# kakaobrain/hqtransformer

Measured on AMD Instinct MI355X. Metric: images/sec (256x256 class-cond sampling), higher is better.
Workload: dtype bf16

## Files before the change

hqtransformer_amd/csrc/common.h:

```cpp
#pragma once
#include <hip/hip_runtime.h>
#include <stdint.h>
#include <string>

typedef uint16_t bf16_t;

__device__ __host__ inline float bf16_to_f32(bf16_t v) {
    union { uint32_t u; float f; } c;
    c.u = ((uint32_t)v) << 16;
    return c.f;
}
__device__ __forceinline__ void bf16x8_to_f32(const uint4& raw, float (&f)[8]) {
    const unsigned w[4] = {raw.x, raw.y, raw.z, raw.w};
#pragma unroll
    for (int i = 0; i < 4; ++i) { f[2 * i] = bf16_to_f32((bf16_t)(w[i] & 0xffffu)); f[2 * i + 1] = bf16_to_f32((bf16_t)(w[i] >> 16)); }
}
__device__ __host__ inline bf16_t f32_to_bf16(float f) {
#if defined(__HIP_DEVICE_COMPILE__)
    return __builtin_bit_cast(bf16_t, (__bf16)f);
#endif
    union { uint32_t u; float f; } c;
    c.f = f;
    if ((c.u & 0x7fffffffu) > 0x7f800000u) return (bf16_t)((c.u >> 16) | 0x40);
    return (bf16_t)((c.u + 0x7fffu + ((c.u >> 16) & 1u)) >> 16);
// ... 87 lines not shown
    float alpha;
    int store;
    int rows_per_group;
    int group_stride;
    int row_offset;
    const int* row_offset_dev;
    int rows_per_image;
    int clamp01;
    void* C2;
    void* C3;
    int qkv_D;
    int qkv_first;
    bf16_t* qkv_v_pk;
    int c_packed_mb;
    const void* zero_page;
    const float* ln_parts;
    int ln_nparts;
    const float* ln_colsum;
    float ln_eps;
    bf16_t* resid_pk;
    float* resid_parts;
    unsigned* tile_ctr;
    const float* am_rownorm;
    const float* am_colnorm;
    unsigned long long* am_best;
    ChainSync chain;
    float* gn_part_out;
    int gn_out_groups;
    int tune;
    const void* Bw_lo;
    const void* Bw_frag16;
    const void* Bw_up16;
    double* gn_part_out_d;
    int a_f32;
    int b_f32;
    int* range_flag;
    int out_split;
    int k_quarters;
    int b_tile16;
    int k_slices;
    float* k_slabs;
    int tile_panel;
    const int* row_pos;
};

__device__ __forceinline__ int row_live(const int* row_pos, int b) { const int p = row_pos[b]; return p < 0 ? 0 : p; }
__device__ __forceinline__ bool row_idle(const int* row_pos, int b) { return row_pos && row_pos[b] < 0; }
__device__ __forceinline__ int qkv_row_of(const GemmArgs& g, int b, int uniform) { return g.row_pos ? row_live(g.row_pos, b) : uniform; }

struct StepState {
    int step;
    int t_base;
};
__device__ __forceinline__ int step_of(const StepState* state, const int* row_pos, int b) { return row_pos ? row_live(row_pos, b) : state->step; }
struct RowKey {
    unsigned long long seed;
    long long global_row;
};
struct RowSampler {
    float temperature[3];
    int top_k[3];
    float top_p[3];
};
struct GuidePair {
    int pos_row, neg_row;
    float scale[3];
};

#define HQT_MAX_V 16384

__device__ __forceinline__ long long clamp_idx(long long v, int n) { return n > 0 ? (v < 0 ? 0 : (v >= n ? (long long)n - 1 : v)) : v; }
```

hqtransformer_amd/csrc/engine.hip:

```cpp
#include "../../include/hqt.h"
#include "kernels.h"
#include "fast_kernels.h"
#include "split_kernels.h"
#include "persist.h"

#include <algorithm>
#include <cmath>
#include <cstdarg>
#include <cstdio>
#include <cstring>
#include <map>
#include <memory>
#include <mutex>
#include <string>
#include <vector>

static thread_local std::string g_err;
static int fail(int code, const char* fmt, ...) {
    char buf[1024];
    va_list ap;
    va_start(ap, fmt);
    vsnprintf(buf, sizeof(buf), fmt, ap);
    va_end(ap);
    g_err = buf;
// ... 134 lines not shown
        int groups_G = 0;
        bool seg = false;
        int seg_start = 0, seg_stop = 0;
        std::vector<int32_t> roll;
        int roll_k = 0;
        bool holds_table() const { return !row_set.empty() || logprob || !guide.empty() || !keep.empty() || !groups.empty(); }
    } staged;
    Staged take_staged() { Staged s = std::move(staged); staged = Staged(); return s; }
    void clear_staged() { staged = Staged(); }
    void *pg_k = nullptr, *pg_v = nullptr;
    float* pg_x = nullptr;
    int pg_cap = 0;
    size_t pg_bytes = 0;
    int max_joins = 0;
    struct Paused { bool live = false; int B = 0, n_steps = 0, levels = 0, precision = 0, pos = 0; } paused;
    struct Rolling { bool live = false; int B = 0, n_steps = 0, levels = 0, precision = 0; std::vector<int32_t> next; } rolling;
    int64_t *cond_buf = nullptr, *codes_top = nullptr, *codes_bot = nullptr;
    int64_t* codes_l2 = nullptr;
    Lin head_l2;
    std::vector<DecLayer> dec;
    std::vector<DecLayer> enc;
    bool has_encoder = false;
    Lin post_quant, quant_conv;
    float* cb_norm[3] = {nullptr, nullptr, nullptr};
    float *vq_h = nullptr, *vq_recon = nullptr, *vq_zz = nullptr, *vq_err = nullptr;
    void* vq_z = nullptr;
    unsigned long long* vq_best = nullptr;
    float* up_table = nullptr;
    Lin up_lin, down_lin;
    float *vq_t = nullptr, *vq_q = nullptr;
    void* act[4] = {nullptr, nullptr, nullptr, nullptr};
    double* gn_partial = nullptr;
    float* gn_tiles = nullptr;
    void* zero_page = nullptr;
    int* range_flag = nullptr;
    size_t act_elems = 0;
    int dec_chunk = 0;
    void *aq = nullptr, *ak = nullptr, *av = nullptr, *ao = nullptr, *as = nullptr, *quant = nullptr;
    float* gn = nullptr;
    hipGraphExec_t graph_exec = nullptr;
    std::vector<uint64_t> graph_key;
    hqt_handle* parent = nullptr;
    int n_clones = 0;
    int policy = 0;
    PersistProg pbody, pfull;
    float* lnf_shift = nullptr;
    int ncu = 0;
    unsigned* persist_counters = nullptr;
    unsigned* persist_err = nullptr;
    float* persist_slabs = nullptr;
    bool persist_used = false;
    bool persist_enabled = true;
    bool persist_tripped = false;
    bool single_key = true;
    bool split_kslices = true;
    bool capture_persist = false;
    bool graph_has_persist = false;
    int layouts = 0;
    bool timing = false;
    std::vector<TimingSlot> slots;
    hipEvent_t chain_ev = nullptr;
    bool chain_valid = false;
    std::vector<hipEvent_t> all_events;
};

static int dev_alloc(hqt_handle* h, void** p, size_t bytes, bool workspace) {
// ... 152 lines not shown
            block_in = block_out;
            if (is_attn_res(label) && c.s1_use_attn)
                add(2, "encoder.down." + std::to_string(lvl) + ".attn." + std::to_string(b), block_in, block_in, res);
        }
        if (lvl != n - 1) {
            add(5, "encoder.down." + std::to_string(lvl) + ".downsample.conv", block_in, block_in, res);
            res /= 2; label /= 2;
        }
    }
    if (c.s1_use_mid_block) {
        add(1, "encoder.mid.block_1", block_in, block_in, res);
        if (c.s1_use_attn) add(2, "encoder.mid.attn_1", block_in, block_in, res);
        add(1, "encoder.mid.block_2", block_in, block_in, res);
    }
    add(7, "encoder", block_in, c.s1_z_channels, res);
}

extern "C" int hqt_abi_version(void) { return HQT_ABI_VERSION; }
extern "C" const char* hqt_last_error(void) { return g_err.c_str(); }

static int alloc_workspace(hqt_handle* hp);

extern "C" int hqt_create(const hqt_config* cfg, int device, hqt_handle** out) {
    if (!cfg || !out) return fail(HQT_ERR_INVALID, "null argument");
    if (cfg->abi_version != HQT_ABI_VERSION) return fail(HQT_ERR_INVALID, "abi_version %d != %d", cfg->abi_version, HQT_ABI_VERSION);
    if (cfg->max_batch < 1) return fail(HQT_ERR_INVALID, "max_batch must be >= 1");
    DeviceGuard dg(device);
    if (!dg.ok) return fail(HQT_ERR_HIP, "hipSetDevice(%d) failed", device);
    std::unique_ptr<hqt_handle> h(new hqt_handle());
    h->tile_gemm = getenv("HQT_NO_TILE_GEMM") == nullptr;
    { const char* e = getenv("HQT_PERSIST"); h->persist_enabled = !(e && atoi(e) == 0); }
    h->single_key = getenv("HQT_NO_SINGLE_KEY") == nullptr;
    h->split_kslices = getenv("HQT_SPLIT_KSLICES_OFF") == nullptr;
    h->cfg = *cfg;
    h->layouts = (cfg->ar_layouts & HQT_LAYOUT_ALL) ? (cfg->ar_layouts & HQT_LAYOUT_ALL) : HQT_LAYOUT_ALL;
    h->device = device;
    const hqt_config& c = h->cfg;
    if (c.has_stage2) {
        if (c.embed_dim % c.n_heads || c.embed_dim % 16) return fail(HQT_ERR_INVALID, "embed_dim must be a multiple of n_heads and 16");
        const int hs = c.embed_dim / c.n_heads;
        if (hs % 8 || hs > 256 || (hs & (hs - 1))) return fail(HQT_ERR_INVALID, "head_dim %d unsupported (power of two in [8, 256])", hs);
        if (c.vocab_top != c.vocab_bot) return fail(HQT_ERR_INVALID, "vocab_top != vocab_bot");
        const bool bidir = c.depth_decoding == HQT_DEPTH_BIDIRECTIONAL;
        if (c.depth_decoding < 0 || c.depth_decoding > HQT_DEPTH_BIDIRECTIONAL || (c.depth_decoding && !bidir && c.code_levels != 3) || (bidir && c.code_levels == 3))
            return fail(HQT_ERR_INVALID, "depth_decoding %d: 0 'parallel-add', 1 'parallel', 2 'parallel-reduce', 3 'top2mid2bot' (three code levels only), "
                        "4 'bidirectional' (two code levels only)", c.depth_decoding);
        if (bidir && c.cond_type == HQT_COND_TEXT)
            return fail(HQT_ERR_INVALID, "depth_decoding 4 'bidirectional' with text conditioning is not built");
        if (c.vocab_top > HQT_MAX_V || c.vocab_top % 4) return fail(HQT_ERR_INVALID, "vocab size %d unsupported", c.vocab_top);
        if (c.cond_type == HQT_COND_CLASS && c.n_classes < 1) return fail(HQT_ERR_INVALID, "n_classes");
        if (c.max_steps < 1 || c.max_steps > c.ctx_len_img) return fail(HQT_ERR_INVALID, "max_steps must be in [1, ctx_len_img]");
    }
    if (c.has_stage1) {
        if (c.s1_n_mult < 1 || c.s1_n_mult > 8) return fail(HQT_ERR_INVALID, "s1_n_mult");
        if (c.s1_ch % 32) return fail(HQT_ERR_INVALID, "GroupNorm(32) needs ch %% 32 == 0");
        if (c.s1_z_channels % 16 || (2 * c.s1_embed_dim) % 16) return fail(HQT_ERR_INVALID, "z_channels and 2*embed_dim must be multiples of 16");
        if (c.s1_resample < 0 || c.s1_resample > HQT_RESAMPLE_CONV2) return fail(HQT_ERR_INVALID, "s1_resample %d: 0 pixelshuffle, 1 nearest, 2 conv2", c.s1_resample);
        if (c.s1_resample && c.code_levels == 3) return fail(HQT_ERR_INVALID, "s1_resample %d with three code levels: the three-level HQ-VAE is built with pixelshuffle only", c.s1_resample);
        if (c.s1_resample == HQT_RESAMPLE_CONV2 && c.s1_embed_dim % 16) return fail(HQT_ERR_INVALID, "s1_resample 2 (conv2) needs embed_dim %% 16 == 0");
        build_decoder_plan(h.get());
        build_encoder_plan(h.get());
    }
    CHK(alloc_workspace(h.get()));
    *out = h.release();
    return HQT_OK;
}
// ... 127 lines not shown
        CHK(dev_alloc(h.get(), (void**)&h->codes_bot, B * (size_t)c.max_steps * 4 * 8, true));
        if (c.code_levels == 3) CHK(dev_alloc(h.get(), (void**)&h->codes_l2, B * (size_t)c.max_steps * 16 * 8, true));
        if (!h->parent) {
            CHK(dev_alloc(h.get(), (void**)&h->persist_counters, PERSIST_COUNTER_BYTES, true));
            CHK(dev_alloc(h.get(), (void**)&h->persist_err, 256, true));
            HIPCHK(hipMemset(h->persist_err, 0, 256));
            CHK(dev_alloc(h.get(), (void**)&h->persist_slabs, persist_slab_floats(256) * 4, true));
        } else {
            h->persist_counters = nullptr; h->persist_err = nullptr; h->persist_slabs = nullptr;
        }
    }
    if (c.has_stage1) {
        std::vector<DecLayer> both(h->dec);
        both.insert(both.end(), h->enc.begin(), h->enc.end());
        size_t per_img = 0;
        for (auto& l : both) {
            const size_t in_e = (size_t)l.res * l.res * (l.kind == 6 ? 16 : l.cin);
            const size_t out_r = l.kind == 3 ? 2 * l.res : l.res;
            const size_t out_e = out_r * out_r * (size_t)(l.kind == 4 ? 0 : l.cout);
            per_img = std::max(per_img, std::max(in_e, out_e));
        }
        h->dec_chunk = std::max(1, std::min<int>(c.max_batch, getenv("HQT_DEC_CHUNK") ? atoi(getenv("HQT_DEC_CHUNK")) : 64));
        h->act_elems = per_img * h->dec_chunk;
        for (int i = 0; i < 3; ++i) CHK(dev_alloc(h.get(), &h->act[i], h->act_elems * 4, true));
        CHK(dev_alloc(h.get(), &h->act[3], h->act_elems * 4, true));
        {
            size_t pe = 0;
            for (auto& l : both) if (l.kind != 6) pe = std::max(pe, gn_stats_fast_partial_elems(h->dec_chunk, l.res * l.res, l.cin, 32));
            for (auto& l : both) if (l.kind == 1) pe = std::max(pe, gn_stats_fast_partial_elems(h->dec_chunk, l.res * l.res, l.cout, 32));
            CHK(dev_alloc(h.get(), (void**)&h->gn_partial, pe * sizeof(double), true));
            size_t te = 0;
            for (auto& l : both) { const int ro = l.kind == 3 ? 2 * l.res : l.res; te = std::max(te, (size_t)h->dec_chunk * (ro / 8 + 1) * (ro / 16 + 1) * 64); }
            CHK(dev_alloc(h.get(), (void**)&h->gn_tiles, te * sizeof(double), true));
        }
        const int r = h->dec.front().res;
        size_t attn_c = 0;
        for (auto& l : both) if (l.kind == 2) attn_c = std::max(attn_c, (size_t)l.cin * l.res * l.res);
        const size_t hw = (size_t)r * r;
        if (attn_c) {
            CHK(dev_alloc(h.get(), &h->aq, attn_c * h->dec_chunk * 4, true));
            CHK(dev_alloc(h.get(), &h->ak, attn_c * h->dec_chunk * 4, true));
            CHK(dev_alloc(h.get(), &h->av, attn_c * h->dec_chunk * 4, true));
            CHK(dev_alloc(h.get(), &h->ao, attn_c * h->dec_chunk * 4, true));
            size_t smax = 0;
            for (auto& l : both) if (l.kind == 2) smax = std::max(smax, (size_t)l.res * l.res * l.res * l.res);
            CHK(dev_alloc(h.get(), &h->as, smax * h->dec_chunk * 4, true));
        }
        CHK(dev_alloc(h.get(), &h->quant, hw * 2 * c.s1_embed_dim * h->dec_chunk * 4, true));
        CHK(dev_alloc(h.get(), (void**)&h->gn, (size_t)h->dec_chunk * 32 * 2 * 2 * 4, true));
        if (h->has_encoder) CHK(alloc_encode_workspace(h.get()));
    }
    return HQT_OK;
}

extern "C" int hqt_clone(hqt_handle* src, hqt_handle** out) {
    if (!src || !out) return fail(HQT_ERR_INVALID, "null argument");
    if (!src->finalized) return fail(HQT_ERR_STATE, "hqt_clone needs a finalized handle");
    ON_DEVICE(src);
    hqt_handle* root = src->parent ? src->parent : src;
    std::unique_ptr<hqt_handle> h(new hqt_handle(*root));
    h->owned.clear();
    h->workspace_bytes = 0;
    h->parent = root;
    h->n_clones = 0;
    h->graph_exec = nullptr;
    h->graph_key.clear();
// ... 1785 lines not shown
        PersistOrder order(h->device, c.st, h->graph_has_persist);
        if (h->graph_has_persist) h->persist_used = true;
        for (int s = 0; s < remaining / G; ++s) HIPCHK(hipGraphLaunch(h->graph_exec, c.st));
        return HQT_OK;
    }
    const bool may_persist = c.md.fast && c.B <= 64 && (persist_on(h, c, h->pfull) || persist_on(h, c, h->pbody));
    PersistOrder order(h->device, c.st, may_persist);
    for (int s = 0; s < remaining; ++s) CHK(run_decode_step(h, c));
    return HQT_OK;
}

static const float* W1(hqt_handle* h, const std::string& name) { return h->w["stage1." + name].d; }

static GemmArgs conv_args(const void* in, int nimg, int res_out, int cin, int taps, int upsample, void* out, int cout) {
    GemmArgs g{};
    g.A = in; g.conv_taps = taps; g.H = res_out; g.W = res_out; g.Cin = cin; g.upsample = upsample;
    g.M = nimg * res_out * res_out; g.batch = 1;
    g.C = out; g.ldc = cout; g.store = STORE_ROWS;
    return g;
}
static void with_gn(GemmArgs& g, const float* stats, const float* gamma, const float* beta, int swish) {
    g.gn_stats = stats; g.gn_gamma = gamma; g.gn_beta = beta; g.gn_groups = 32; g.gn_swish = swish;
}

struct S1Ctx {
    hqt_handle* h;
    int n;
    Mode md;
    hipStream_t st;
    int adt;
    void *cur, *t1, *t2, *tn;
    float *gn1, *gn2;
    bool cur_planes = false;
    struct { const void* tensor; int tiles; bool dbl; } gn_ready = {nullptr, 0, false};
};

enum S1Operand { S1_TENSOR, S1_PLANES, S1_SPLIT_IN_KERNEL };

static bool split_shape_ok(const hqt_handle* h, const GemmArgs& g, const Lin& l) {
    if (!l.w16h) return false;
    GemmArgs t = g;
    lin_args(h, t, l, true);
    return t.conv_taps == 9 ? split_conv3_ok(t) : split_gemm_ok(t);
}
static int s1_split_pack(S1Ctx& c, GemmArgs* g, const float* stats, const float* gamma, const float* beta, int swish) {
    hqt_handle* h = c.h;
    const int hw_in = g->conv_taps ? ((g->H << g->conv_stride2) >> g->upsample) * ((g->W << g->conv_stride2) >> g->upsample) : 0;
    const int C = g->conv_taps ? g->Cin : g->lda;
    const int rows = g->conv_taps ? c.n : 1, per = g->conv_taps ? hw_in : g->M;
    Timed t(h, "split_pack", c.st);
    HIPCHK(launch_split_pack(reinterpret_cast<const float*>(g->A), reinterpret_cast<half_t*>(c.tn), stats, gamma, beta, rows, per, C, 32, swish, h->range_flag, c.st));
    g->A = c.tn;
    if (!g->conv_taps) g->lda = 2 * C;
    return HQT_OK;
}

static int s1_split_stats(S1Ctx& c, const void* src, int C, int hw, float* stats) {
    Timed t(c.h, "gn_stats", c.st);
    if (c.gn_ready.tensor == src && c.gn_ready.dbl) {
        count_variant(c.h, "variant:gn_stats_tiles:gn");
        HIPCHK(launch_gn_finalize_tiles_d(reinterpret_cast<const double*>(c.h->gn_tiles), stats, c.n, c.gn_ready.tiles, hw, C, 32, 1e-6f, c.st));
    } else {
        count_variant(c.h, "variant:gn_stats_pass:gn");
        HIPCHK(launch_gn_stats_fast(src, stats, c.h->gn_partial, c.n, hw, C, 32, 1e-6f, c.st, DT_F32));
    }
    return HQT_OK;
}

static int s1_norm(S1Ctx& c, const void* src, int C, int hw, float* stats, const float* gamma, const float* beta, int swish, GemmArgs* g,
                   const Lin& l, S1Operand* a) {
    hqt_handle* h = c.h;
    hipStream_t st = c.st;
    *a = S1_TENSOR;
    if (c.md.fast) {
        {
            Timed t(h, "gn_stats", st);
            if (c.gn_ready.tensor == src && !c.gn_ready.dbl) {
                count_variant(h, "variant:gn_stats_tiles:gn");
                HIPCHK(launch_gn_finalize_tiles(h->gn_tiles, stats, c.n, c.gn_ready.tiles, hw, C, 32, 1e-6f, st));
            } else {
                count_variant(h, "variant:gn_stats_pass:gn");
                HIPCHK(launch_gn_stats_fast(src, stats, h->gn_partial, c.n, hw, C, 32, 1e-6f, st));
            }
        }
        { Timed t(h, "gn_apply", st); HIPCHK(launch_gn_apply(src, c.tn, stats, gamma, beta, c.n, hw, C, 32, swish, st)); }
        g->A = c.tn;
    } else if (c.md.split && split_shape_ok(h, *g, l)) {
        CHK(s1_split_stats(c, src, C, hw, stats));
        CHK(s1_split_pack(c, g, stats, gamma, beta, swish));
        *a = S1_PLANES;
    } else {
        { Timed t(h, "gn_stats", st); HIPCHK(launch_gn_stats(src, c.adt, stats, c.n, hw, C, 32, 1e-6f, st)); }
        count_variant(h, "variant:gn_stats_two_pass:gn");
        with_gn(*g, stats, gamma, beta, swish);
    }
    return HQT_OK;
}
static int s1_plain(S1Ctx& c, GemmArgs* g, const Lin& l, S1Operand* a) {
    *a = S1_TENSOR;
    if (!c.md.split) return HQT_OK;
    if (g->conv_taps == 1) {
        GemmArgs t = *g;
        t.a_f32 = 1;
        if (split_shape_ok(c.h, t, l)) {
            g->a_f32 = 1; g->range_flag = c.h->range_flag; *a = S1_SPLIT_IN_KERNEL;
            return HQT_OK;
        }
    }
    if (!split_shape_ok(c.h, *g, l)) return HQT_OK;
    *a = S1_PLANES;
    return s1_split_pack(c, g, nullptr, nullptr, nullptr, 0);
}

static int s1_conv(S1Ctx& c, GemmArgs g, S1Operand a, const Lin& l, int c_dt, const char* tag) {
    hqt_handle* h = c.h;
    lin_args(h, g, l, a != S1_TENSOR);
    Timed t(h, SlotName(tag, g.M).s, c.st);
    if (c.gn_ready.tensor == g.C) c.gn_ready.tensor = nullptr;
    if (a != S1_TENSOR) {
        if (g.conv_taps != 9) { count_variant(h, "variant:split_gemm:%s", tag); HIPCHK(launch_split_gemm(g, c.st)); return HQT_OK; }
        count_variant(h, "variant:split_conv3:%s", tag);
        if (g.store == STORE_ROWS && h->gn_tiles && conv_halo_stats_ok(g.N, 32)) {
            g.gn_part_out_d = reinterpret_cast<double*>(h->gn_tiles); g.gn_out_groups = 32;
            c.gn_ready = {g.C, split_conv3_tiles_per_image(g), true};
        }
        HIPCHK(launch_split_conv3(g, c.st));
        return HQT_OK;
    }
    if (c.md.fast) {
        g.Bw = l.w16;
        if (!mfma_gemm_ok(g, c.adt, DT_BF16, c_dt)) {
            count_variant(h, "variant:gemm_generic_bf16:%s", tag);
            HIPCHK(launch_gemm_generic(g, c.adt, DT_BF16, c_dt, c.st));
            return HQT_OK;
        }
        if (h->timing) count_variant(h, conv_halo_ok(g, c_dt) ? "variant:halo_conv:%s" : "variant:mfma_gemm:%s", tag);
        if (g.conv_taps == 9 && g.store == STORE_ROWS && h->gn_tiles && conv_halo_ok(g, c_dt) && conv_halo_stats_ok(g.N, 32) &&
            !getenv("HQT_NO_FUSED_GN")) {
            g.gn_part_out = h->gn_tiles; g.gn_out_groups = 32;
            c.gn_ready = {g.C, conv_halo_tiles_per_image(g), false};
        }
        HIPCHK(launch_mfma_gemm(g, c.adt, DT_BF16, c_dt, c.st));
        return HQT_OK;
    }
    g.Bw = l.w32;
    count_variant(h, "variant:gemm_generic_f32:%s", tag);
    HIPCHK(launch_gemm_generic(g, DT_F32, DT_F32, DT_F32, c.st));
    return HQT_OK;
}

static bool s1_split_product(hqt_handle* h, const Mode& md, GemmArgs& sg) {
    if (!md.split) return false;
    GemmArgs t = sg;
    t.a_f32 = 1; t.b_f32 = 1; t.range_flag = h->range_flag;
    if (!split_gemm_ok(t)) return false;
    sg = t;
    return true;
}

static int s1_layer(S1Ctx& c, const DecLayer& l, const DecLayer* next = nullptr) {
    hqt_handle* h = c.h;
    hipStream_t st = c.st;
    const int adt = c.adt, n = c.n;
    void *&cur = c.cur, *&t1 = c.t1, *&t2 = c.t2;
    const int res = l.res, hw = res * res;
    if (l.kind == 0 || l.kind == 3) {
        const int ro = l.kind == 3 ? 2 * res : res;
        GemmArgs g = conv_args(cur, n, ro, l.cin, 9, l.kind == 3, t1, l.cout);
        S1Operand a = S1_PLANES;
        if (c.cur_planes) c.cur_planes = false;
        else CHK(s1_plain(c, &g, l.conv1, &a));
        CHK(s1_conv(c, g, a, l.conv1, adt, "conv3x3"));
        std::swap(cur, t1);
// ... 87 lines not shown
        Timed t(h, "quant_gather", st);
        if (l3) {
            QuantArgs3 q{code_t, code_m, code_b, seq_layout, W1(h, "quantizers.0.embedding"), W1(h, "quantizers.1.embedding"),
                         W1(h, "quantizers.2.embedding"), h->quant, n, r, E, adt, cf.s1_n_embed};
            HIPCHK(launch_quant_gather3(q, st));
        } else if (cf.s1_resample) {
            const bool conv2 = cf.s1_resample == HQT_RESAMPLE_CONV2;
            QuantRowsArgs q{code_t, code_b, seq_layout, conv2 ? h->up_table : W1(h, "quantize_t.embedding"), conv2 ? 4 : 1,
                            conv2 ? W1(h, "upsample_t.bias") : nullptr, W1(h, "quantize_b.embedding"), h->quant, n, r, E, adt, cf.s1_n_embed};
            HIPCHK(launch_quant_gather_rows(q, st));
        } else {
            QuantArgs q{code_t, code_b, seq_layout, W1(h, "quantize_t.embedding"), W1(h, "quantize_b.embedding"), h->quant, n, r, E, adt, cf.s1_n_embed};
            HIPCHK(launch_quant_gather(q, st));
        }
    }
    S1Ctx c{h, n, md, st, adt, h->act[0], h->act[1], h->act[2], h->act[3], h->gn, h->gn + (size_t)h->dec_chunk * 64};
    {
        GemmArgs g = conv_args(h->quant, n, r, l3 ? E : 2 * E, 1, 0, c.cur, cf.s1_z_channels);
        S1Operand a;
        CHK(s1_plain(c, &g, h->post_quant, &a));
        CHK(s1_conv(c, g, a, h->post_quant, adt, "conv1x1"));
    }
    for (size_t li = 0; li < h->dec.size(); ++li) {
        const DecLayer& l = h->dec[li];
        if (l.kind != 4) { CHK(s1_layer(c, l, li + 1 < h->dec.size() ? &h->dec[li + 1] : nullptr)); continue; }
        const int hw = l.res * l.res;
        GemmArgs g = conv_args(c.cur, n, l.res, l.cin, 9, 0, out, l.cout);
        g.store = STORE_NCHW; g.rows_per_image = hw; g.clamp01 = clamp01;
        if (md.split && l.conv1.w32) {
            GemmArgs d = g;
            d.N = l.conv1.N; d.K = l.conv1.K; d.Bw = l.conv1.w32; d.bias = l.conv1.b32; d.alpha = 1.0f;
            with_gn(d, c.gn1, l.n1_g, l.n1_b, 1);
            if (conv_out_direct_ok(d)) {
                CHK(s1_split_stats(c, c.cur, l.cin, hw, c.gn1));
                Timed t(h, "conv_out", st);
                HIPCHK(launch_conv_out_direct(d, st));
                count_variant(h, "variant:conv_out_direct:conv_out");
                continue;
            }
        }
        S1Operand a;
        CHK(s1_norm(c, c.cur, l.cin, hw, c.gn1, l.n1_g, l.n1_b, 1, &g, l.conv1, &a));
        CHK(s1_conv(c, g, a, l.conv1, DT_F32, "conv_out"));
    }
    return HQT_OK;
}

static int decode_impl(hqt_handle* h, int B, const int64_t* code_t, const int64_t* code_m, const int64_t* code_b, int seq_layout, float* out,
                       int clamp01, int precision, void* stream, int levels) {
    if (!h || !out) return fail(HQT_ERR_INVALID, "null argument");
    if (!h->finalized) return fail(HQT_ERR_STATE, "hqt_finalize_weights has not run");
    if (!h->cfg.has_stage1) return fail(HQT_ERR_STATE, "handle was created without stage 1");
    if ((h->cfg.code_levels == 3) != (levels == 3)) return fail(HQT_ERR_STATE, "stage 1 has %d code levels: use the matching decode entry point", h->cfg.code_levels == 3 ? 3 : 2);
    if (!code_t && !code_b && !code_m) return fail(HQT_ERR_INVALID, "every code grid is NULL");
    if (B < 1) return fail(HQT_ERR_INVALID, "B must be >= 1");
    ON_DEVICE(h);
    Mode md;
    CHK(mode_of(precision, true, &md));
    const int r = h->dec.front().res;
    const int rt = levels == 3 ? r / 4 : r / 2, rm = r / 2;
    const size_t out_per = (size_t)h->cfg.s1_out_ch * h->dec.back().res * h->dec.back().res;
    for (int b0 = 0; b0 < B; b0 += h->dec_chunk) {
        const int n = std::min(h->dec_chunk, B - b0);
        const int64_t* ct = code_t ? code_t + (size_t)b0 * rt * rt : nullptr;
        const int64_t* cm = code_m ? code_m + (size_t)b0 * rm * rm : nullptr;
        const int64_t* cb = code_b ? code_b + (size_t)b0 * r * r : nullptr;
        CHK(decode_chunk(h, n, ct, cm, cb, seq_layout, out + (size_t)b0 * out_per, clamp01, md, (hipStream_t)stream));
// ... 211 lines not shown
```

hqtransformer_amd/csrc/kernels.hip:

```cpp
#include "kernels.h"
#include <mutex>
#include "gemm_generic.h"
#include <type_traits>

template <typename T, typename Op>
__device__ __forceinline__ T wave_reduce(T v, Op op) {
#pragma unroll
    for (int off = 32; off > 0; off >>= 1) v = op(v, __shfl_xor(v, off, 64));
    return v;
}
template <typename T, typename Op>
__device__ __forceinline__ T block_reduce(T v, Op op, T* scratch ) {
    v = wave_reduce(v, op);
    const int wid = threadIdx.x >> 6, nw = blockDim.x >> 6;
    __syncthreads();
    if ((threadIdx.x & 63) == 0) scratch[wid] = v;
    __syncthreads();
    T r = scratch[0];
    for (int i = 1; i < nw; ++i) r = op(r, scratch[i]);
    return r;
}
struct OpAdd { template <typename T> __device__ T operator()(T a, T b) const { return a + b; } };
struct OpMax { template <typename T> __device__ T operator()(T a, T b) const { return a > b ? a : b; } };
struct OpMin { template <typename T> __device__ T operator()(T a, T b) const { return a < b ? a : b; } };
// ... 1505 lines not shown
    for (int c = threadIdx.x; c < C; c += 256) {
        float ts = 0.0f, tq = 0.0f;
        for (int r = 0; r < rpi; ++r) { ts += part[(size_t)r * C + c]; tq += part[(size_t)(rpi + r) * C + c]; }
        part[(size_t)2 * rpi * C + c] = ts;
        part[(size_t)2 * rpi * C + C + c] = tq;
    }
    __syncthreads();
    const float* tot = part + (size_t)2 * rpi * C;
    const int cpg = C / groups;
    for (int g = threadIdx.x; g < groups; g += 256) {
        double a = 0.0, c2 = 0.0;
        for (int i = 0; i < cpg; ++i) { a += (double)tot[g * cpg + i]; c2 += (double)tot[C + g * cpg + i]; }
        partial[((long long)blockIdx.x * groups + g) * 2] = a;
        partial[((long long)blockIdx.x * groups + g) * 2 + 1] = c2;
    }
}
__global__ void gn_finalize_kernel(const double* partial, float* stats, int nchunk, int groups, double count, float eps, int n) {
    const int bg = blockIdx.x * blockDim.x + threadIdx.x;
    if (bg >= n) return;
    const int b = bg / groups, g = bg % groups;
    double a = 0.0, q = 0.0;
    for (int ch = 0; ch < nchunk; ++ch) {
        a += partial[(((long long)b * nchunk + ch) * groups + g) * 2];
        q += partial[(((long long)b * nchunk + ch) * groups + g) * 2 + 1];
    }
    const double mean = a / count;
    const double var = fmax(q / count - mean * mean, 0.0);
    stats[(long long)bg * 2] = (float)mean;
    stats[(long long)bg * 2 + 1] = (float)(1.0 / sqrt(var + (double)eps));
}
template <typename TP>
__global__ __launch_bounds__(64) void gn_finalize_tiles_kernel(const TP* partial, float* stats, int tiles, int groups, double count, float eps) {
    const int bg = blockIdx.x;
    const int b = bg / groups, g = bg % groups;
    double a = 0.0, q = 0.0;
    for (int t = threadIdx.x; t < tiles; t += 64) {
        const TP* p = partial + (((long long)b * tiles + t) * groups + g) * 2;
        a += (double)p[0];
        q += (double)p[1];
    }
    a = wave_reduce(a, OpAdd());
    q = wave_reduce(q, OpAdd());
    if (threadIdx.x == 0) {
        const double mean = a / count;
        const double var = fmax(q / count - mean * mean, 0.0);
        stats[(long long)bg * 2] = (float)mean;
        stats[(long long)bg * 2 + 1] = (float)(1.0 / sqrt(var + (double)eps));
    }
}
hipError_t launch_gn_finalize_tiles(const float* partial, float* stats, int B, int tiles, int HW, int C, int groups, float eps, hipStream_t st) {
    gn_finalize_tiles_kernel<float><<<B * groups, 64, 0, st>>>(partial, stats, tiles, groups, (double)HW * (C / groups), eps);
    return hipGetLastError();
}
hipError_t launch_gn_finalize_tiles_d(const double* partial, float* stats, int B, int tiles, int HW, int C, int groups, float eps, hipStream_t st) {
    gn_finalize_tiles_kernel<double><<<B * groups, 64, 0, st>>>(partial, stats, tiles, groups, (double)HW * (C / groups), eps);
    return hipGetLastError();
}
size_t gn_stats_fast_partial_elems(int B, int HW, int C, int groups) {
    (void)C;
    const int cp = gn_chunk_pix(HW);
    return (size_t)B * ((HW + cp - 1) / cp) * groups * 2;
}
hipError_t launch_gn_stats_fast(const void* x, float* stats, double* partial, int B, int HW, int C, int groups, float eps,
                                hipStream_t st, int dtype) {
    const int cp = gn_chunk_pix(HW);
    const int nchunk = (HW + cp - 1) / cp;
    if (gn_fixed_ok(C)) {
        const int rpi = 256 / (C / 8);
        const size_t smem = (size_t)(2 * rpi + 2) * C * sizeof(float);
        if (dtype == DT_F32) gn_partial_kernel<float><<<B * nchunk, 256, smem, st>>>((const float*)x, partial, HW, C, groups, nchunk, cp);
        else gn_partial_kernel<bf16_t><<<B * nchunk, 256, smem, st>>>((const bf16_t*)x, partial, HW, C, groups, nchunk, cp);
    } else {
        const size_t smem = (size_t)(2 * gn_generic_rpi(C) + 2) * C * sizeof(float);
        if (C % 8 != 0 || smem > 64 * 1024) return hipErrorInvalidValue;
        if (dtype == DT_F32) gn_partial_generic_kernel<float><<<B * nchunk, 256, smem, st>>>((const float*)x, partial, HW, C, groups, nchunk, cp);
        else gn_partial_generic_kernel<bf16_t><<<B * nchunk, 256, smem, st>>>((const bf16_t*)x, partial, HW, C, groups, nchunk, cp);
    }
    hipError_t e = hipGetLastError();
    if (e != hipSuccess) return e;
    const int n = B * groups;
    gn_finalize_kernel<<<(n + 63) / 64, 64, 0, st>>>(partial, stats, nchunk, groups, (double)HW * (C / groups), eps, n);
// ... 330 lines not shown
```

hqtransformer_amd/csrc/split_conv.hip:

```cpp
#include "split_kernels.h"
#include "split_ring.h"
#include "gemm_generic.h"
#include <algorithm>
#include <cstdlib>
#include <type_traits>

namespace {
__device__ __forceinline__ unsigned pack_h2(half_t a, half_t b) {
    return (unsigned)__builtin_bit_cast(unsigned short, a) | ((unsigned)__builtin_bit_cast(unsigned short, b) << 16);
}

__device__ __forceinline__ void xcd_tile(int& tile_m, int& tile_n) {
    const int nx = gridDim.x, total = gridDim.x * gridDim.y;
    int id = blockIdx.x + nx * blockIdx.y;
    if ((total & 7) == 0) id = (id & 7) * (total >> 3) + (id >> 3);
    tile_m = id / nx;
    tile_n = id - tile_m * nx;
}
}

__global__ void split_f32_kernel(const float* __restrict__ src, half_t* __restrict__ hi, half_t* __restrict__ lo, size_t n) {
    for (size_t i = blockIdx.x * (size_t)blockDim.x + threadIdx.x; i < n; i += (size_t)gridDim.x * blockDim.x) split2(src[i], hi[i], lo[i]);
}
hipError_t launch_split_f32(const float* src, half_t* hi, half_t* lo, size_t n, hipStream_t st) {
// ... 291 lines not shown
                    if (n >= g.N) continue;
                    float v = (accm[i][j][e] + accx[i][j][e] * SPLIT_INV) * g.alpha + (g.bias ? g.bias[n] : 0.0f);
                    if (g.clamp01) v = fminf(fmaxf(0.5f * v + 0.5f, 0.0f), 1.0f);
                    Cb[((long long)img * g.N + n) * hw + pix] = v;
                }
        }
        return;
    }
    if constexpr (BN == 128) {
        const long long pix0 = ((long long)img * g.H + ty0) * g.W + tx0;
        char* stage = lds_raw;
        float gs[8], gq[8];
#pragma unroll
        for (int e = 0; e < 8; ++e) { gs[e] = 0.0f; gq[e] = 0.0f; }
        if (consumer) {
#pragma unroll
        for (int i = 0; i < FI; ++i) {
            const int r = wm * 64 + i * 32 + fr;
#pragma unroll
            for (int j = 0; j < 2; ++j)
#pragma unroll
                for (int q4 = 0; q4 < 4; ++q4) {
                    const int nl = wn * 64 + j * 32 + 8 * q4 + 4 * fh;
                    f32x4 v;
#pragma unroll
                    for (int e = 0; e < 4; ++e) v[e] = accm[i][j][4 * q4 + e] + accx[i][j][4 * q4 + e] * SPLIT_INV;
                    *reinterpret_cast<f32x4*>(stage + r * S_CPITCH + nl * 4) = v;
                }
        }
        }
        __syncthreads();
        ring_store_rows<8>(g, stage, tid, n0, bv, consumer, [&](int r) { return pix0 + (long long)(r >> 4) * g.W + (r & 15); }, gs, gq);
        ring_reduce_gn(g, lds_raw, tid, gs, gq, n0, consumer, (long long)img * (tiles_x * tiles_y) + trem);
    }
}

bool split_conv3_ok(const GemmArgs& g) {
    if (g.conv_taps != 9 || g.conv_stride2 || g.conv_nopad || !g.zero_page || g.gn_stats || g.a_packed_mb || g.batch > 1) return false;
    if (!g.Bw_lo || g.ldb % 8 != 0 || g.K != 9 * g.Cin || g.M % (g.H * g.W) != 0) return false;
    if (g.Cin % 64 != 0 || g.H % S_TY != 0 || g.W % S_TX != 0) return false;
    if (g.act != ACT_NONE) return false;
    if (g.store == STORE_NCHW) return !g.resid && g.N <= 32;
    return g.store == STORE_ROWS && g.rows_per_group == 0 && g.ldc % 8 == 0 && g.N % 8 == 0;
}
int split_conv3_tiles_per_image(const GemmArgs& g) { return split_stream_ok(g) ? split_stream_tiles_per_image(g) : (g.H / S_TY) * (g.W / S_TX); }
hipError_t launch_split_conv3(const GemmArgs& g, hipStream_t st) {
    if (split_stream_ok(g)) return launch_split_conv3_stream(g, st);
    if (g.store == STORE_NCHW) conv3x3_split_kernel<true, 32, 1><<<dim3(1, g.M / (S_TY * S_TX), 1), 512, split_conv3_lds(32), st>>>(g);
    else conv3x3_split_kernel<false, 128, 1><<<dim3((g.N + 127) / 128, g.M / (S_TY * S_TX), 1), 512, split_conv3_lds(128), st>>>(g);
    return hipGetLastError();
}

template <bool AF32, bool BF32>
__global__ __launch_bounds__(256, 2) void split_gemm_kernel(GemmArgs g, int a_lo_off) {
    constexpr int BM = 128, BN = 128, BKG = 32, ROWB = 64, OPB = 128 * ROWB;
    extern __shared__ __attribute__((aligned(16))) char lds_raw[];
    auto LDS = [&](int stage, int op) -> char* { return lds_raw + (size_t)(stage * 4 + op) * OPB; };
    const int tid = threadIdx.x, lane = tid & 63, wave = tid >> 6;
    const int wm = wave >> 1, wn = wave & 1;
    const int S = (AF32 && !BF32 && g.k_slices > 1) ? g.k_slices : 1;
    const int ks = S > 1 ? (int)blockIdx.z : 0, bz = S > 1 ? 0 : (int)blockIdx.z;
    const int kbase = ks * (g.K / S);
    int tile_m, tile_n;
    xcd_tile(tile_m, tile_n);
    const int m0 = tile_m * BM, n0 = tile_n * BN;
    const half_t* Abase = reinterpret_cast<const half_t*>(g.A) + (long long)bz * g.a_batch_stride;
// ... 358 lines not shown
```

hqtransformer_amd/csrc/split_ring.h:

```cpp
#pragma once
#include "split_kernels.h"
#include "split_device.h"

typedef _Float16 half8 __attribute__((ext_vector_type(8)));
typedef __attribute__((ext_vector_type(16))) float f32x16;
typedef __attribute__((ext_vector_type(4))) float f32x4;
typedef __attribute__((ext_vector_type(4))) unsigned int u32x4;

namespace {
constexpr float R_INV = 1.0f / 2048.0f;
constexpr int R_TY = 8, R_TX = 16, R_PITCH = R_TX + 2;
constexpr int R_ROWS = (R_TY + 2) * R_PITCH;
constexpr int R_PIECES = (R_ROWS + 15) / 16;
constexpr int R_PPW = 2 * R_PIECES / 4;
constexpr int R_CPITCH = 128 * 4 + 16;
static_assert(R_PPW == 6, "one piece per wave at taps 0..5");
constexpr int G_PITCH = 80, G_PLANE = 16 * R_PIECES * G_PITCH, G_LDS = 4 * G_PLANE;
static_assert(64 * R_CPITCH <= G_LDS, "epilogue staging (64 pixels at a time) must fit in the patch buffers");
static_assert(3 * G_PLANE + 38 * G_PITCH + 32 < 65536, "ds_read immediate offsets");

constexpr int H_RING = 3, H_AHEAD = H_RING - 1, H_STEPS = 18;
static_assert(H_STEPS % H_RING == 0, "static ring slots");
constexpr bool h_piece_at(int u) { u = ((u % H_STEPS) + H_STEPS) % H_STEPS; return (u % 9) < 6; }
constexpr int h_younger(int s, int per_step = 4) {
    int n = per_step * (H_AHEAD - 1);
    for (int u = s - H_AHEAD; u < s; ++u) n += h_piece_at(u) ? 1 : 0;
    return n;
}

__device__ __forceinline__ void r_xcd_tile(int& tile_m, int& tile_n, int panel) {
    const int nx = gridDim.x, total = gridDim.x * gridDim.y;
    int id = blockIdx.x + nx * blockIdx.y;
    if ((total & 7) == 0) id = (id & 7) * (total >> 3) + (id >> 3);
    if (panel > 0) {
        const int per = panel * nx, p = id / per, r = id - p * per;
        const int rows = min(panel, (int)gridDim.y - p * panel);
        tile_n = r / rows;
        tile_m = p * panel + (r - tile_n * rows);
        return;
    }
// ... 122 lines not shown
            }
        }
    }
}
template <int PASSES, class PixelOf>
__device__ __forceinline__ void ring_store_rows(const GemmArgs& g, const char* stage, int tid, int n0, const float (&bv)[8], bool active,
                                                PixelOf pixel_of, float (&gs)[8], float (&gq)[8]) {
    bool bad = false;
    ring_store_rows<PASSES, false>(g, stage, tid, n0, bv, active, pixel_of, gs, gq, bad);
}
__device__ __forceinline__ void ring_reduce_gn(const GemmArgs& g, char* lds_raw, int tid, const float (&gs)[8], const float (&gq)[8], int n0,
                                               bool active, long long part) {
    if (!g.gn_part_out_d) return;
    const int c8 = (tid & 15) * 8;
    __syncthreads();
    float* redw = reinterpret_cast<float*>(lds_raw);
    if (active) {
#pragma unroll
        for (int e = 0; e < 8; ++e) {
            redw[(((tid >> 4) * 128) + c8 + e) * 2] = gs[e];
            redw[(((tid >> 4) * 128) + c8 + e) * 2 + 1] = gq[e];
        }
    }
    __syncthreads();
    const float* red = reinterpret_cast<const float*>(lds_raw);
    if (active && tid < 128) {
        double sa = 0.0, sq = 0.0;
#pragma unroll
        for (int rg = 0; rg < 16; ++rg) { sa += (double)red[((rg * 128) + tid) * 2]; sq += (double)red[((rg * 128) + tid) * 2 + 1]; }
        const int cpg = g.N / g.gn_out_groups;
        for (int off = cpg >> 1; off > 0; off >>= 1) { sa += __shfl_xor(sa, off, 64); sq += __shfl_xor(sq, off, 64); }
        const int ch = n0 + tid;
        if (ch < g.N && (tid & (cpg - 1)) == 0) {
            double* pp = g.gn_part_out_d + (part * g.gn_out_groups + ch / cpg) * 2;
            pp[0] = sa; pp[1] = sq;
        }
    }
}
}
```

hqtransformer_amd/csrc/split_stream_conv.hip:

```cpp
#include "split_kernels.h"
#include "split_ring.h"
#include "gemm_generic.h"
#include <algorithm>
#include <cstdlib>
#include <type_traits>

constexpr size_t R_FRAG_PAD = 3 * 4 * 512;
size_t split_frag_elems(int N, int Cin) { return (size_t)((N + 31) / 32) * (Cin / 32) * 9 * 4 * 512 + R_FRAG_PAD; }

__global__ void pack_split_frag16_kernel(const float* __restrict__ w, half_t* __restrict__ out, int N, int Cin, size_t total) {
    const int NC = Cin / 32;
    for (size_t i = blockIdx.x * (size_t)blockDim.x + threadIdx.x; i < total; i += (size_t)gridDim.x * blockDim.x) {
        const int j = (int)(i & 7), lane = (int)((i >> 3) & 63);
        size_t ch = i >> 9;
        const int plane = (int)(ch & 1); ch >>= 1;
        const int blk = (int)(ch & 1); ch >>= 1;
        const int tap = (int)(ch % 9); ch /= 9;
        const int c = (int)(ch % NC);
        const int t = (int)(ch / NC);
        const int n = t * 32 + blk * 16 + (lane & 15), k = tap * Cin + c * 32 + 8 * (lane >> 4) + j;
        const float x = n < N ? w[(size_t)n * 9 * Cin + k] : 0.0f;
        const half_t hi = (half_t)x;
        out[i] = plane ? (half_t)((x - (float)hi) * 2048.0f) : hi;
    }
// ... 115 lines not shown
                    if (pr == 0 && ABL != 5) ring_load_b4(wh[nslot], wl[nslot], lane16, bfrag, S + H_AHEAD);
                    if (pr == 1 && ABL != 2) {
                        if (tap >= 2 && tap - 2 < R_PPW) {
                            if (tap - 1 < R_PPW) asm volatile("s_waitcnt vmcnt(9)" : "+v"(pst[tap % 2]));
                            else asm volatile("s_waitcnt vmcnt(8)" : "+v"(pst[tap % 2]));
                            ring_store_piece(piece_base, pst[tap % 2], cc ^ 1, tap - 2);
                        }
                        if (tap < R_PPW) ring_load_piece(pst[tap % 2], poff, img_rsrc, cn, tap, g.Cin);
                    }
                }
            }
        }
    }
    asm volatile("s_waitcnt vmcnt(0) lgkmcnt(0)" ::: "memory");
    __builtin_amdgcn_s_barrier();
    __builtin_amdgcn_sched_barrier(0);
    if (ABL == 1) { ring_sink_acc(g, accm, accx); return; }
    const long long pix0 = ((long long)img * g.H + ty0) * g.W + tx0;
    char* stage = lds_raw;
    float bv[8], gs[8], gq[8];
    ring_bias8(g, n0 + (tid & 15) * 8, bv);
    bool bad = false;
#pragma unroll
    for (int e = 0; e < 8; ++e) { gs[e] = 0.0f; gq[e] = 0.0f; }
#pragma unroll
    for (int half = 0; half < 2; ++half) {
        if (half > 0) __syncthreads();
        h_stage_half(stage, accm, accx, half, wave, fx, fk);
        __syncthreads();
        ring_store_rows<4, true>(g, stage, tid, n0, bv, true, [&](int r) { return pix0 + (long long)(half * 4 + (r >> 4)) * g.W + (r & 15); }, gs, gq, bad);
    }
    if (bad && g.range_flag) atomicOr(g.range_flag, 1);
    ring_reduce_gn(g, lds_raw, tid, gs, gq, n0, true, (long long)img * (tiles_x * tiles_y) + trem);
}


__global__ void pack_split_up16_kernel(const float* __restrict__ w, half_t* __restrict__ out, int N, int Cin, size_t total) {
    const int NC = Cin / 32, NG = (N + 31) / 32;
    for (size_t i = blockIdx.x * (size_t)blockDim.x + threadIdx.x; i < total; i += (size_t)gridDim.x * blockDim.x) {
        const int j = (int)(i & 7), lane = (int)((i >> 3) & 63);
        size_t ch = i >> 9;
        const int plane = (int)(ch & 1); ch >>= 1;
        const int blk = (int)(ch & 1); ch >>= 1;
        const int tap = (int)(ch & 3); ch >>= 2;
        const int c = (int)(ch % NC); ch /= NC;
        const int t = (int)(ch % NG);
        const int phase = (int)(ch / NG);
        const int pa = phase >> 1, pb = phase & 1, ty = tap >> 1, tx = tap & 1;
        const int n = t * 32 + blk * 16 + (lane & 15), kin = c * 32 + 8 * (lane >> 4) + j;
        const int ky0 = pa == 0 ? (ty == 0 ? 0 : 1) : (ty == 0 ? 0 : 2), ky1 = pa == 0 ? (ty == 0 ? 0 : 2) : (ty == 0 ? 1 : 2);
        const int kx0 = pb == 0 ? (tx == 0 ? 0 : 1) : (tx == 0 ? 0 : 2), kx1 = pb == 0 ? (tx == 0 ? 0 : 2) : (tx == 0 ? 1 : 2);
        double x = 0.0;
        if (n < N)
            for (int ky = ky0; ky <= ky1; ++ky)
                for (int kx = kx0; kx <= kx1; ++kx) x += (double)w[(size_t)n * 9 * Cin + (size_t)(ky * 3 + kx) * Cin + kin];
        const half_t hi = (half_t)(float)x;
        out[i] = plane ? (half_t)(float)((x - (double)(float)hi) * 2048.0) : hi;
    }
}
size_t split_up_elems(int N, int Cin) { return (size_t)4 * ((N + 31) / 32) * (Cin / 32) * 4 * 2048 + 2048; }
hipError_t launch_pack_split_up16(const float* w_tapmajor, half_t* out, int N, int Cin, hipStream_t st) {
    const size_t total = split_up_elems(N, Cin) - 2048;
    pack_split_up16_kernel<<<(int)std::min<size_t>((total + 255) / 256, 8192), 256, 0, st>>>(w_tapmajor, out, N, Cin, total);
    return hipGetLastError();
}

// ... 93 lines not shown
                    }
                    if (pr < 2) {
                        if (pr == 0) { ring_read_a16(ah, al, abase, cc, tapoff, 4); ring_read_a16(ah, al, abase, cc, tapoff, 5); }
                        else { ring_read_a16(ah, al, abase, cc, tapoff, 6); ring_read_a16(ah, al, abase, cc, tapoff, 7); }
                    } else if (tap < TAPS - 1) {
                        if (pr == 2) { ring_read_a16(ah, al, abase, cc, ntapoff, 0); ring_read_a16(ah, al, abase, cc, ntapoff, 1); }
                        else { ring_read_a16(ah, al, abase, cc, ntapoff, 2); ring_read_a16(ah, al, abase, cc, ntapoff, 3); }
                    }
                    if (pr >= 1 && tap < 2 && ABL != 2) ring_load_piece(pst[3 * tap + pr - 1], poff, img_rsrc, cn, 3 * tap + pr - 1, g.Cin);
                }
            }
        }
    }
    asm volatile("s_waitcnt vmcnt(0) lgkmcnt(0)" ::: "memory");
    __builtin_amdgcn_s_barrier();
    __builtin_amdgcn_sched_barrier(0);
    if (ABL == 1) { ring_sink_acc(g, accm, accx); return; }
    char* stage = lds_raw;
    float bv[8], gs[8], gq[8];
    ring_bias8(g, n0 + (tid & 15) * 8, bv);
#pragma unroll
    for (int e = 0; e < 8; ++e) { gs[e] = 0.0f; gq[e] = 0.0f; }
#pragma unroll
    for (int half = 0; half < 2; ++half) {
        if (half > 0) __syncthreads();
        h_stage_half(stage, accm, accx, half, wave, fx, fk);
        __syncthreads();
        ring_store_rows<4>(g, stage, tid, n0, bv, true, [&](int r) {
            const long long oy = 2 * (ty0 + half * 4 + (r >> 4)) + pa, ox = 2 * (tx0 + (r & 15)) + pb;
            return ((long long)img * g.H + oy) * g.W + ox;
        }, gs, gq);
    }
    ring_reduce_gn(g, lds_raw, tid, gs, gq, n0, true, ((long long)img * (tiles_x * tiles_y) + trem) * 4 + phase);
}


__global__ __launch_bounds__(256, 2) void conv3x3_split_out16_kernel(GemmArgs g) {
    extern __shared__ __attribute__((aligned(16))) char lds_raw[];
    const unsigned lds_base = (unsigned)(size_t)(__attribute__((address_space(3))) char*)lds_raw;
    const int tid = threadIdx.x, lane = tid & 63;
    const int wave = __builtin_amdgcn_readfirstlane(tid >> 6);
    const int fx = lane & 15, fk = lane >> 4;
    const int tile_m = blockIdx.y;
    int img, trem, ty0, tx0, tiles_x, tiles_y;
    ring_tile(tile_m, g.H, g.W, img, trem, ty0, tx0, tiles_x, tiles_y);
    const int Hin = g.H >> g.upsample, Win = g.W >> g.upsample;
    const int NC = g.Cin / 32;

    const ring_rsrc_t img_rsrc = ring_image_rsrc(g.A, img, Hin, Win, g.Cin);
    unsigned poff[3];
    ring_piece_offsets(poff, wave, lane, ty0, tx0, g.H, g.W, Win, g.upsample, g.Cin);
    u32x4 pst[2];
    unsigned piece_base = ring_piece_base(lds_base, wave, lane);

    const char* bfrag = reinterpret_cast<const char*>(g.Bw_frag16);
    unsigned lane16 = lane * 16;

    f32x4 accm[2], accx[2];
#pragma unroll
    for (int i = 0; i < 2; ++i)
#pragma unroll
        for (int r = 0; r < 4; ++r) { accm[i][r] = 0.0f; accx[i][r] = 0.0f; }
    const unsigned abase = ring_frag_base(lds_base, 2 * wave * R_PITCH + fx, fk);
    half8 ah[4], al[4];
    half8 wh[H_RING], wl[H_RING];

// ... 211 lines not shown
```

Baseline: 1704.

## Finalize GroupNorm stats inside split conv via last-arriving-block ticket

Split conv kernels now write GN partials with agent-scope atomic stores and bump a per-image arrival counter. The last block to arrive for an image computes the mean and rstd for all groups and writes them to a stats buffer. The host then skips the separate gn_finalize launch when those stats are ready. This removes one kernel launch and its serialization per GroupNorm, at the cost of an extra barrier and atomic in every conv block plus a serial tail on the last block.

Result: no change. 1699 (-0.2%).

```diff
diff --git a/hqtransformer_amd/csrc/common.h b/hqtransformer_amd/csrc/common.h
--- a/hqtransformer_amd/csrc/common.h
+++ b/hqtransformer_amd/csrc/common.h
@@ -143,6 +143,9 @@
     const void* Bw_frag16;
     const void* Bw_up16;
     double* gn_part_out_d;
+    unsigned* gn_arrive;
+    float* gn_stats_out;
+    float gn_out_eps;
     int a_f32;
     int b_f32;
     int* range_flag;
@@ -159,6 +162,26 @@
 __device__ __forceinline__ bool row_idle(const int* row_pos, int b) { return row_pos && row_pos[b] < 0; }
 __device__ __forceinline__ int qkv_row_of(const GemmArgs& g, int b, int uniform) { return g.row_pos ? row_live(g.row_pos, b) : uniform; }
 
+template <typename TP>
+__device__ __forceinline__ void gn_tiles_mean_rstd(const TP* partial, float* stats, int b, int g, int tiles, int groups, double count, float eps, int lane) {
+    double a = 0.0, q = 0.0;
+    for (int t = lane; t < tiles; t += 64) {
+        const TP* p = partial + (((long long)b * tiles + t) * groups + g) * 2;
+        a += (double)p[0];
+        q += (double)p[1];
+    }
+#pragma unroll
+    for (int off = 32; off > 0; off >>= 1) a += __shfl_xor(a, off, 64);
+#pragma unroll
+    for (int off = 32; off > 0; off >>= 1) q += __shfl_xor(q, off, 64);
+    if (lane == 0) {
+        const double mean = a / count;
+        const double var = fmax(q / count - mean * mean, 0.0);
+        stats[((long long)b * groups + g) * 2] = (float)mean;
+        stats[((long long)b * groups + g) * 2 + 1] = (float)(1.0 / sqrt(var + (double)eps));
+    }
+}
+
 struct StepState {
     int step;
     int t_base;
diff --git a/hqtransformer_amd/csrc/engine.hip b/hqtransformer_amd/csrc/engine.hip
--- a/hqtransformer_amd/csrc/engine.hip
+++ b/hqtransformer_amd/csrc/engine.hip
@@ -190,6 +190,9 @@
     void* act[4] = {nullptr, nullptr, nullptr, nullptr};
     double* gn_partial = nullptr;
     float* gn_tiles = nullptr;
+    unsigned* gn_arrive = nullptr;
+    float* gn_fin = nullptr;
+    bool gn_in_conv = true;
     void* zero_page = nullptr;
     int* range_flag = nullptr;
     size_t act_elems = 0;
@@ -408,6 +411,7 @@
     { const char* e = getenv("HQT_PERSIST"); h->persist_enabled = !(e && atoi(e) == 0); }
     h->single_key = getenv("HQT_NO_SINGLE_KEY") == nullptr;
     h->split_kslices = getenv("HQT_SPLIT_KSLICES_OFF") == nullptr;
+    { const char* e = getenv("HQT_GN_FINALIZE_LAUNCH"); h->gn_in_conv = !(e && atoi(e) != 0); }
     h->cfg = *cfg;
     h->layouts = (cfg->ar_layouts & HQT_LAYOUT_ALL) ? (cfg->ar_layouts & HQT_LAYOUT_ALL) : HQT_LAYOUT_ALL;
     h->device = device;
@@ -601,6 +605,10 @@
             size_t te = 0;
             for (auto& l : both) { const int ro = l.kind == 3 ? 2 * l.res : l.res; te = std::max(te, (size_t)h->dec_chunk * (ro / 8 + 1) * (ro / 16 + 1) * 64); }
             CHK(dev_alloc(h.get(), (void**)&h->gn_tiles, te * sizeof(double), true));
+            CHK(dev_alloc(h.get(), (void**)&h->gn_fin, (size_t)h->dec_chunk * 32 * 2 * 4, true));
+            CHK(dev_alloc(h.get(), (void**)&h->gn_arrive, (size_t)h->dec_chunk * 4, true));
+            HIPCHK(hipMemset(h->gn_arrive, 0, (size_t)h->dec_chunk * 4));
+            HIPCHK(hipDeviceSynchronize());
         }
         const int r = h->dec.front().res;
         size_t attn_c = 0;
@@ -2452,7 +2460,7 @@
     void *cur, *t1, *t2, *tn;
     float *gn1, *gn2;
     bool cur_planes = false;
-    struct { const void* tensor; int tiles; bool dbl; } gn_ready = {nullptr, 0, false};
+    struct { const void* tensor; int tiles; bool dbl; const float* stats; } gn_ready = {nullptr, 0, false, nullptr};
 };
 
 enum S1Operand { S1_TENSOR, S1_PLANES, S1_SPLIT_IN_KERNEL };
@@ -2475,7 +2483,13 @@
     return HQT_OK;
 }
 
-static int s1_split_stats(S1Ctx& c, const void* src, int C, int hw, float* stats) {
+static int s1_split_stats(S1Ctx& c, const void* src, int C, int hw, float* stats, const float** use) {
+    *use = stats;
+    if (c.gn_ready.tensor == src && c.gn_ready.dbl && c.gn_ready.stats) {
+        count_variant(c.h, "variant:gn_stats_tiles:gn");
+        *use = c.gn_ready.stats;
+        return HQT_OK;
+    }
     Timed t(c.h, "gn_stats", c.st);
     if (c.gn_ready.tensor == src && c.gn_ready.dbl) {
         count_variant(c.h, "variant:gn_stats_tiles:gn");
@@ -2506,8 +2520,9 @@
         { Timed t(h, "gn_apply", st); HIPCHK(launch_gn_apply(src, c.tn, stats, gamma, beta, c.n, hw, C, 32, swish, st)); }
         g->A = c.tn;
     } else if (c.md.split && split_shape_ok(h, *g, l)) {
-        CHK(s1_split_stats(c, src, C, hw, stats));
-        CHK(s1_split_pack(c, g, stats, gamma, beta, swish));
+        const float* use;
+        CHK(s1_split_stats(c, src, C, hw, stats, &use));
+        CHK(s1_split_pack(c, g, use, gamma, beta, swish));
         *a = S1_PLANES;
     } else {
         { Timed t(h, "gn_stats", st); HIPCHK(launch_gn_stats(src, c.adt, stats, c.n, hw, C, 32, 1e-6f, st)); }
@@ -2542,7 +2557,11 @@
         count_variant(h, "variant:split_conv3:%s", tag);
         if (g.store == STORE_ROWS && h->gn_tiles && conv_halo_stats_ok(g.N, 32)) {
             g.gn_part_out_d = reinterpret_cast<double*>(h->gn_tiles); g.gn_out_groups = 32;
-            c.gn_ready = {g.C, split_conv3_tiles_per_image(g), true};
+            c.gn_ready = {g.C, split_conv3_tiles_per_image(g), true, nullptr};
+            if (h->gn_in_conv) {
+                g.gn_arrive = h->gn_arrive; g.gn_stats_out = h->gn_fin; g.gn_out_eps = 1e-6f;
+                c.gn_ready.stats = h->gn_fin;
+            }
         }
         HIPCHK(launch_split_conv3(g, c.st));
         return HQT_OK;
@@ -2558,7 +2577,7 @@
         if (g.conv_taps == 9 && g.store == STORE_ROWS && h->gn_tiles && conv_halo_ok(g, c_dt) && conv_halo_stats_ok(g.N, 32) &&
             !getenv("HQT_NO_FUSED_GN")) {
             g.gn_part_out = h->gn_tiles; g.gn_out_groups = 32;
-            c.gn_ready = {g.C, conv_halo_tiles_per_image(g), false};
+            c.gn_ready = {g.C, conv_halo_tiles_per_image(g), false, nullptr};
         }
         HIPCHK(launch_mfma_gemm(g, c.adt, DT_BF16, c_dt, c.st));
         return HQT_OK;
@@ -2712,7 +2731,7 @@
             d.N = l.conv1.N; d.K = l.conv1.K; d.Bw = l.conv1.w32; d.bias = l.conv1.b32; d.alpha = 1.0f;
             with_gn(d, c.gn1, l.n1_g, l.n1_b, 1);
             if (conv_out_direct_ok(d)) {
-                CHK(s1_split_stats(c, c.cur, l.cin, hw, c.gn1));
+                CHK(s1_split_stats(c, c.cur, l.cin, hw, c.gn1, &d.gn_stats));
                 Timed t(h, "conv_out", st);
                 HIPCHK(launch_conv_out_direct(d, st));
                 count_variant(h, "variant:conv_out_direct:conv_out");
diff --git a/hqtransformer_amd/csrc/kernels.hip b/hqtransformer_amd/csrc/kernels.hip
--- a/hqtransformer_amd/csrc/kernels.hip
+++ b/hqtransformer_amd/csrc/kernels.hip
@@ -1561,21 +1561,7 @@
 template <typename TP>
 __global__ __launch_bounds__(64) void gn_finalize_tiles_kernel(const TP* partial, float* stats, int tiles, int groups, double count, float eps) {
     const int bg = blockIdx.x;
-    const int b = bg / groups, g = bg % groups;
-    double a = 0.0, q = 0.0;
-    for (int t = threadIdx.x; t < tiles; t += 64) {
-        const TP* p = partial + (((long long)b * tiles + t) * groups + g) * 2;
-        a += (double)p[0];
-        q += (double)p[1];
-    }
-    a = wave_reduce(a, OpAdd());
-    q = wave_reduce(q, OpAdd());
-    if (threadIdx.x == 0) {
-        const double mean = a / count;
-        const double var = fmax(q / count - mean * mean, 0.0);
-        stats[(long long)bg * 2] = (float)mean;
-        stats[(long long)bg * 2 + 1] = (float)(1.0 / sqrt(var + (double)eps));
-    }
+    gn_tiles_mean_rstd(partial, stats, bg / groups, bg % groups, tiles, groups, count, eps, (int)threadIdx.x);
 }
 hipError_t launch_gn_finalize_tiles(const float* partial, float* stats, int B, int tiles, int HW, int C, int groups, float eps, hipStream_t st) {
     gn_finalize_tiles_kernel<float><<<B * groups, 64, 0, st>>>(partial, stats, tiles, groups, (double)HW * (C / groups), eps);
diff --git a/hqtransformer_amd/csrc/split_conv.hip b/hqtransformer_amd/csrc/split_conv.hip
--- a/hqtransformer_amd/csrc/split_conv.hip
+++ b/hqtransformer_amd/csrc/split_conv.hip
@@ -347,6 +347,8 @@
         __syncthreads();
         ring_store_rows<8>(g, stage, tid, n0, bv, consumer, [&](int r) { return pix0 + (long long)(r >> 4) * g.W + (r & 15); }, gs, gq);
         ring_reduce_gn(g, lds_raw, tid, gs, gq, n0, consumer, (long long)img * (tiles_x * tiles_y) + trem);
+        static_assert(S_TY * S_TX == R_TY * R_TX, "ring_finish_gn counts a partial as one ring tile's pixels");
+        ring_finish_gn(g, lds_raw, tid, consumer, img, tiles_x * tiles_y, tiles_x * tiles_y * (int)gridDim.x);
     }
 }
 
diff --git a/hqtransformer_amd/csrc/split_ring.h b/hqtransformer_amd/csrc/split_ring.h
--- a/hqtransformer_amd/csrc/split_ring.h
+++ b/hqtransformer_amd/csrc/split_ring.h
@@ -6,6 +6,8 @@
 typedef __attribute__((ext_vector_type(16))) float f32x16;
 typedef __attribute__((ext_vector_type(4))) float f32x4;
 typedef __attribute__((ext_vector_type(4))) unsigned int u32x4;
+typedef __attribute__((address_space(1))) unsigned long long gn_word_t;
+typedef __attribute__((address_space(1))) unsigned gn_ctr_t;
 
 namespace {
 constexpr float R_INV = 1.0f / 2048.0f;
@@ -194,9 +196,34 @@
         for (int off = cpg >> 1; off > 0; off >>= 1) { sa += __shfl_xor(sa, off, 64); sq += __shfl_xor(sq, off, 64); }
         const int ch = n0 + tid;
         if (ch < g.N && (tid & (cpg - 1)) == 0) {
-            double* pp = g.gn_part_out_d + (part * g.gn_out_groups + ch / cpg) * 2;
-            pp[0] = sa; pp[1] = sq;
-        }
-    }
-}
-}
+            gn_word_t* pp = (gn_word_t*)g.gn_part_out_d + (part * g.gn_out_groups + ch / cpg) * 2;
+            __hip_atomic_store(pp, (unsigned long long)__double_as_longlong(sa), __ATOMIC_RELAXED, __HIP_MEMORY_SCOPE_AGENT);
+            __hip_atomic_store(pp + 1, (unsigned long long)__double_as_longlong(sq), __ATOMIC_RELAXED, __HIP_MEMORY_SCOPE_AGENT);
+        }
+    }
+}
+__device__ __forceinline__ void ring_finish_gn(const GemmArgs& g, char* lds_raw, int tid, bool active, int img, int tiles, int arrivals) {
+    if (!g.gn_arrive) return;
+    asm volatile("s_waitcnt vmcnt(0)" ::: "memory");
+    __syncthreads();
+    volatile __attribute__((address_space(3))) unsigned* ticket = (volatile __attribute__((address_space(3))) unsigned*)lds_raw;
+    if (active && tid == 0) {
+        gn_ctr_t* ctr = (gn_ctr_t*)g.gn_arrive + img;
+        const unsigned t = __hip_atomic_fetch_add(ctr, 1u, __ATOMIC_RELAXED, __HIP_MEMORY_SCOPE_AGENT);
+        if (t + 1u == (unsigned)arrivals) {
+            __hip_atomic_store(ctr, 0u, __ATOMIC_RELAXED, __HIP_MEMORY_SCOPE_AGENT);
+            __builtin_amdgcn_fence(__ATOMIC_ACQUIRE, "agent");
+            asm volatile("s_waitcnt vmcnt(0)" ::: "memory");
+        }
+        ticket[0] = t;
+    }
+    __syncthreads();
+    if (ticket[0] + 1u != (unsigned)arrivals || !active || tid >= 256) return;
+    const double count = (double)(tiles * (R_TY * R_TX)) * (g.N / g.gn_out_groups);
+    const int per_wave = (g.gn_out_groups + 3) / 4;
+    for (int k = 0; k < per_wave; ++k) {
+        const int grp = (tid >> 6) * per_wave + k;
+        if (grp < g.gn_out_groups) gn_tiles_mean_rstd(g.gn_part_out_d, g.gn_stats_out, img, grp, tiles, g.gn_out_groups, count, g.gn_out_eps, tid & 63);
+    }
+}
+}
diff --git a/hqtransformer_amd/csrc/split_stream_conv.hip b/hqtransformer_amd/csrc/split_stream_conv.hip
--- a/hqtransformer_amd/csrc/split_stream_conv.hip
+++ b/hqtransformer_amd/csrc/split_stream_conv.hip
@@ -171,6 +171,7 @@
     }
     if (bad && g.range_flag) atomicOr(g.range_flag, 1);
     ring_reduce_gn(g, lds_raw, tid, gs, gq, n0, true, (long long)img * (tiles_x * tiles_y) + trem);
+    ring_finish_gn(g, lds_raw, tid, true, img, tiles_x * tiles_y, tiles_x * tiles_y * (int)gridDim.x);
 }
 
 
@@ -330,6 +331,7 @@
         }, gs, gq);
     }
     ring_reduce_gn(g, lds_raw, tid, gs, gq, n0, true, ((long long)img * (tiles_x * tiles_y) + trem) * 4 + phase);
+    ring_finish_gn(g, lds_raw, tid, true, img, 4 * tiles_x * tiles_y, tiles_x * tiles_y * (int)gridDim.x);
 }
 
 
```
